# hirofumi0810/tensorflow_end2end_speech_recognition

Hardware: AMD Instinct MI355X
Metric: acoustic frames/sec (train), TIMIT-shaped BLSTM-CTC (higher is better)
Workload: dtype bf16; 1 GPU; TIMIT 61-phone 5x256 BLSTM-CTC, B=16/GPU, D=120, C=62, seq_len~U{100..778}, dropout 0.2, rmsprop, train step; global_batch=16, parallelism=dp1, padded_to=own Tmax per rank

## Files before the change

tensorflow_end2end_speech_recognition_amd/csrc/gemm.hip:

```cpp
#include "common.h"
#include "mfma_tn.h"
#include <stdlib.h>

namespace {

static inline bool first_on_device(unsigned long long& mask) {
  int d = 0;
  (void)hipGetDevice(&d);
  const unsigned long long bit = 1ull << (d & 63);
  if (mask & bit) return false;
  mask |= bit;
  return true;
}

template <typename T> struct GT;
template <> struct GT<float> {
  static constexpr int BK = 32;
  static constexpr int VEC = 4;
};
template <> struct GT<bf16_t> {
  static constexpr int BK = 64;
  static constexpr int VEC = 8;
};

template <typename T> struct Vec16 { T v[GT<T>::VEC]; } __attribute__((aligned(16)));

template <typename TO> __device__ __forceinline__ void store_out(TO* p, float v);
template <> __device__ __forceinline__ void store_out<float>(float* p, float v) { *p = v; }
template <> __device__ __forceinline__ void store_out<bf16_t>(bf16_t* p, float v) { *p = f32_to_bf16(v); }
template <typename TO> __device__ __forceinline__ float load_out(const TO* p);
template <> __device__ __forceinline__ float load_out<float>(const float* p) { return *p; }
template <> __device__ __forceinline__ float load_out<bf16_t>(const bf16_t* p) { return bf16_to_f32(*p); }

template <typename T, int ROWS, bool KCONT>
struct TileLoader {
  static constexpr int BK = GT<T>::BK, VEC = GT<T>::VEC;
  static constexpr int NVEC = ROWS * BK / VEC;
  static constexpr int PER_THREAD = NVEC / 256;
  static_assert(NVEC % 256 == 0, "tile must divide over 256 threads");
  Vec16<T> reg[PER_THREAD];

  __device__ __forceinline__ void load(const T* __restrict__ p, int ld, int r0, int k0, int R,
                                       int K, bool aligned) {
    const int tid = threadIdx.x;
#pragma unroll
    for (int i = 0; i < PER_THREAD; ++i) {
      const int v = tid + i * 256;
      int r, k;
      size_t off;
      int nr, nk;
      if (KCONT) {
        r = v / (BK / VEC); k = (v % (BK / VEC)) * VEC;
        off = (size_t)(r0 + r) * ld + (k0 + k);
        nr = 1; nk = VEC;
      } else {
        k = v / (ROWS / VEC); r = (v % (ROWS / VEC)) * VEC;
        off = (size_t)(k0 + k) * ld + (r0 + r);
        nr = VEC; nk = 1;
      }
      const bool full = (r0 + r + nr <= R) && (k0 + k + nk <= K);
      if (full && aligned) {
        reg[i] = *reinterpret_cast<const Vec16<T>*>(p + off);
      } else {
#pragma unroll
        for (int j = 0; j < VEC; ++j) {
          const int rr = r0 + r + (KCONT ? 0 : j), kk = k0 + k + (KCONT ? j : 0);
          T val = T(0);
          if (rr < R && kk < K) val = p[KCONT ? ((size_t)rr * ld + kk) : ((size_t)kk * ld + rr)];
          reg[i].v[j] = val;
        }
      }
    }
  }
  __device__ __forceinline__ void store(T* s, int lds_ld) const {
    const int tid = threadIdx.x;
#pragma unroll
    for (int i = 0; i < PER_THREAD; ++i) {
      const int v = tid + i * 256;
      if (KCONT) {
        const int r = v / (BK / VEC), k = (v % (BK / VEC)) * VEC;
        *reinterpret_cast<Vec16<T>*>(s + r * lds_ld + k) = reg[i];
      } else {
        const int k = v / (ROWS / VEC), r = (v % (ROWS / VEC)) * VEC;
#pragma unroll
        for (int j = 0; j < VEC; ++j) s[(r + j) * lds_ld + k] = reg[i].v[j];
      }
    }
  }
};

template <typename T, typename TO, int BM, int BN, bool TA, bool TB>
__global__ __launch_bounds__(256) void gemm_kernel(int M, int N, int K, const T* __restrict__ A,
                                                   int lda, const T* __restrict__ B, int ldb,
                                                   TO* __restrict__ C, int ldc,
                                                   const float* __restrict__ bias, int accumulate,
                                                   int a_aligned, int b_aligned, int kchunk,
                                                   float* __restrict__ partial, int act, int c_vec) {
  constexpr int BK = GT<T>::BK, VEC = GT<T>::VEC;
  constexpr int LDS_LD = BK + VEC;
  constexpr int WM = BM / 2, WN = BN / 2, TM = WM / 16, TN = WN / 16;
  extern __shared__ __attribute__((aligned(16))) char smem[];
  T* As = reinterpret_cast<T*>(smem);
  T* Bs = As + BM * LDS_LD;

  const int lane = threadIdx.x & 63, wave = threadIdx.x >> 6;
  const int wm = wave >> 1, wn = wave & 1;
  const int m0 = blockIdx.y * BM, n0 = blockIdx.x * BN;

  TileLoader<T, BM, !TA> la;
  TileLoader<T, BN, TB> lb;

  f32x4_t acc[TM][TN];
#pragma unroll
  for (int i = 0; i < TM; ++i)
#pragma unroll
    for (int j = 0; j < TN; ++j) acc[i][j] = (f32x4_t){0.f, 0.f, 0.f, 0.f};

  const int kbeg = blockIdx.z * kchunk;
  const int kend = min(K, kbeg + kchunk);
  const int nkt = (kend - kbeg + BK - 1) / BK;
  constexpr int STAGE = (BM + BN) * LDS_LD;
  la.load(A, lda, m0, kbeg, M, kend, a_aligned);
  lb.load(B, ldb, n0, kbeg, N, kend, b_aligned);
  la.store(As, LDS_LD);
  lb.store(Bs, LDS_LD);
  __syncthreads();

  for (int kt = 0; kt < nkt; ++kt) {
    const T* Ac = As + (kt & 1) * STAGE;
    const T* Bc = Bs + (kt & 1) * STAGE;
    if (kt + 1 < nkt) {
      la.load(A, lda, m0, kbeg + (kt + 1) * BK, M, kend, a_aligned);
      lb.load(B, ldb, n0, kbeg + (kt + 1) * BK, N, kend, b_aligned);
    }
    const int fr = lane & 15, fq = lane >> 4;
    if constexpr (sizeof(T) == 2) {
#pragma unroll
      for (int ks = 0; ks < BK / 32; ++ks) {
        bf16x8_t a[TM], b[TN];
#pragma unroll
        for (int i = 0; i < TM; ++i)
          a[i] = *reinterpret_cast<const bf16x8_t*>(Ac + (wm * WM + i * 16 + fr) * LDS_LD + ks * 32 + fq * 8);
#pragma unroll
        for (int j = 0; j < TN; ++j)
          b[j] = *reinterpret_cast<const bf16x8_t*>(Bc + (wn * WN + j * 16 + fr) * LDS_LD + ks * 32 + fq * 8);
#pragma unroll
        for (int i = 0; i < TM; ++i)
#pragma unroll
          for (int j = 0; j < TN; ++j)
            acc[i][j] = __builtin_amdgcn_mfma_f32_16x16x32_bf16(b[j], a[i], acc[i][j], 0, 0, 0);
      }
    } else {
#pragma unroll
      for (int ks = 0; ks < BK / 4; ++ks) {
        float a[TM], b[TN];
#pragma unroll
        for (int i = 0; i < TM; ++i) a[i] = Ac[(wm * WM + i * 16 + fr) * LDS_LD + ks * 4 + fq];
#pragma unroll
        for (int j = 0; j < TN; ++j) b[j] = Bc[(wn * WN + j * 16 + fr) * LDS_LD + ks * 4 + fq];
#pragma unroll
        for (int i = 0; i < TM; ++i)
#pragma unroll
          for (int j = 0; j < TN; ++j)
            acc[i][j] = __builtin_amdgcn_mfma_f32_16x16x4f32(b[j], a[i], acc[i][j], 0, 0, 0);
      }
    }
    if (kt + 1 < nkt) {
      la.store(As + ((kt + 1) & 1) * STAGE, LDS_LD);
      lb.store(Bs + ((kt + 1) & 1) * STAGE, LDS_LD);
    }
    __syncthreads();
  }

#pragma unroll
  for (int i = 0; i < TM; ++i)
#pragma unroll
    for (int j = 0; j < TN; ++j) {
      const int m = m0 + wm * WM + i * 16 + (lane & 15);
      const int nb = n0 + wn * WN + j * 16 + (lane >> 4) * 4;
      if (m >= M || nb >= N) continue;
      const bool full = nb + 3 < N;
      if (partial) {
        float* pp = partial + ((size_t)blockIdx.z * M + m) * N + nb;
        if (full && (N & 3) == 0) *reinterpret_cast<f32x4_t*>(pp) = acc[i][j];
        else
          for (int r = 0; r < 4 && nb + r < N; ++r) pp[r] = acc[i][j][r];
        continue;
      }
      TO* cp = C + (size_t)m * ldc + nb;
      float v[4];
#pragma unroll
      for (int r = 0; r < 4; ++r) v[r] = acc[i][j][r] + ((bias && nb + r < N) ? bias[nb + r] : 0.f);
      if (full && c_vec) {
        if constexpr (sizeof(TO) == 4) {
          if (accumulate) {
            const f32x4_t o = *reinterpret_cast<const f32x4_t*>(cp);
#pragma unroll
            for (int r = 0; r < 4; ++r) v[r] += o[r];
          }
          if (act == 1) {
#pragma unroll
            for (int r = 0; r < 4; ++r) v[r] = fmaxf(v[r], 0.f);
          }
          *reinterpret_cast<f32x4_t*>(cp) = (f32x4_t){v[0], v[1], v[2], v[3]};
        } else {
          typedef __attribute__((ext_vector_type(4))) unsigned short us4_t;
          if (accumulate) {
            const us4_t o = *reinterpret_cast<const us4_t*>(cp);
#pragma unroll
            for (int r = 0; r < 4; ++r) v[r] += bf16_to_f32(o[r]);
          }
          if (act == 1) {
#pragma unroll
            for (int r = 0; r < 4; ++r) v[r] = fmaxf(v[r], 0.f);
          }
          *reinterpret_cast<us4_t*>(cp) = (us4_t){f32_to_bf16(v[0]), f32_to_bf16(v[1]), f32_to_bf16(v[2]), f32_to_bf16(v[3])};
        }
      } else {
        for (int r = 0; r < 4 && nb + r < N; ++r) {
          float w = v[r];
          if (accumulate) w += load_out<TO>(cp + r);
          if (act == 1) w = fmaxf(w, 0.f);
          store_out<TO>(cp + r, w);
        }
      }
    }
}

__device__ __forceinline__ unsigned nt_swz(int row) { return (((row + 4) >> 3) & 1) ? 8u : 0u; }

template <bool ANY> __device__ __forceinline__ int nt_tile_of_block(int b, int total) {
  if constexpr (ANY) {
    const int per = total >> 3, rem = total & 7, x = b & 7;
    return x * per + min(x, rem) + (b >> 3);
  } else {
    int t = b;
    if ((total & 7) == 0) t = (t & 7) * (total >> 3) + (t >> 3);
    return t;
  }
}

struct GemmDrop {
  float keep;
  uint64_t seed, offset;
  int use;
};

template <typename TO, bool ROWS = false>
__global__ __launch_bounds__(256) void gemm_nt_bf16_kernel(int M, int N, int K, const bf16_t* __restrict__ A,
                                                           int lda, const bf16_t* __restrict__ Bt, int ldb,
                                                           TO* __restrict__ C, int ldc,
                                                           const float* __restrict__ bias, int accumulate,
                                                           int act, const float* __restrict__ mul, int ldm,
                                                           GemmDrop drop, const int32_t* __restrict__ rows) {
  constexpr int BM = 128, BN = 128, BK = 64, LD = BK + 8;
  constexpr int STAGE = (BM + BN) * LD;
  extern __shared__ __attribute__((aligned(16))) char smem[];
  bf16_t* S = reinterpret_cast<bf16_t*>(smem);

  const int tid = threadIdx.x, lane = tid & 63, wave = tid >> 6;
  const int wm = wave >> 1, wn = wave & 1;
  const int ntn = N / BN, ntm = (M + BM - 1) / BM, total = ntn * ntm;
  const int t = nt_tile_of_block<ROWS>((int)blockIdx.x, total);
  const int m0 = (t / ntn) * BM, n0 = (t % ntn) * BN;

  const bf16_t* pa[4];
  const bf16_t* pb[4];
  unsigned so[4];
#pragma unroll
  for (int i = 0; i < 4; ++i) {
    const int v = tid + i * 256, r = v >> 3, kv = (v & 7) * 8;
    const int ar = min(m0 + r, M - 1);
    pa[i] = A + (size_t)(ROWS ? rows[ar] : ar) * lda + kv;
    pb[i] = Bt + (size_t)(n0 + r) * ldb + kv;
    so[i] = (unsigned)(r * LD) + ((unsigned)kv ^ nt_swz(r));
  }
  bf16x8_t ra[4], rb[4];
  auto gload = [&]() {
#pragma unroll
    for (int i = 0; i < 4; ++i) {
      ra[i] = *reinterpret_cast<const bf16x8_t*>(pa[i]);
      rb[i] = *reinterpret_cast<const bf16x8_t*>(pb[i]);
      pa[i] += BK;
      pb[i] += BK;
    }
  };
  auto sstore = [&](bf16_t* st) {
#pragma unroll
    for (int i = 0; i < 4; ++i) {
      *reinterpret_cast<bf16x8_t*>(st + so[i]) = ra[i];
      *reinterpret_cast<bf16x8_t*>(st + BM * LD + so[i]) = rb[i];
    }
  };

  f32x4_t acc[4][4];
#pragma unroll
  for (int i = 0; i < 4; ++i)
#pragma unroll
    for (int j = 0; j < 4; ++j) acc[i][j] = (f32x4_t){0.f, 0.f, 0.f, 0.f};

  const int nkt = K / BK;
  gload();
  sstore(S);
  __syncthreads();
  const int fr = lane & 15, fq = lane >> 4;
  const unsigned aoff = (unsigned)((wm * 64 + fr) * LD) + ((unsigned)(fq * 8) ^ nt_swz(fr));
  const unsigned boff = (unsigned)(BM * LD + (wn * 64 + fr) * LD) + ((unsigned)(fq * 8) ^ nt_swz(fr));
  for (int kt = 0; kt < nkt; ++kt) {
    const bf16_t* cur = S + (kt & 1) * STAGE;
    if (kt + 1 < nkt) gload();
#pragma unroll
    for (int ks = 0; ks < 2; ++ks) {
      bf16x8_t a[4], b[4];
#pragma unroll
      for (int i = 0; i < 4; ++i) a[i] = *reinterpret_cast<const bf16x8_t*>(cur + aoff + i * 16 * LD + ks * 32);
#pragma unroll
      for (int j = 0; j < 4; ++j) b[j] = *reinterpret_cast<const bf16x8_t*>(cur + boff + j * 16 * LD + ks * 32);
#pragma unroll
      for (int i = 0; i < 4; ++i)
#pragma unroll
        for (int j = 0; j < 4; ++j)
          acc[i][j] = __builtin_amdgcn_mfma_f32_16x16x32_bf16(b[j], a[i], acc[i][j], 0, 0, 0);
    }
    if (kt + 1 < nkt) sstore(S + ((kt + 1) & 1) * STAGE);
    __syncthreads();
  }
#pragma unroll
  for (int i = 0; i < 4; ++i) {
    const int mi = m0 + wm * 64 + i * 16 + fr;
    if (mi >= M) continue;
    const int m = ROWS ? rows[mi] : mi;
#pragma unroll
    for (int j = 0; j < 4; ++j) {
      const int nb = n0 + wn * 64 + j * 16 + fq * 4;
      TO* cp = C + (size_t)m * ldc + nb;
      float v[4];
#pragma unroll
      for (int r = 0; r < 4; ++r) v[r] = acc[i][j][r];
      if (bias) {
        const f32x4_t bv = *reinterpret_cast<const f32x4_t*>(bias + nb);
#pragma unroll
        for (int r = 0; r < 4; ++r) v[r] += bv[r];
      }
      if constexpr (sizeof(TO) == 4) {
        if (accumulate) {
          const f32x4_t o = *reinterpret_cast<const f32x4_t*>(cp);
#pragma unroll
          for (int r = 0; r < 4; ++r) v[r] += o[r];
        }
        if (act == 1) {
#pragma unroll
          for (int r = 0; r < 4; ++r) v[r] = fmaxf(v[r], 0.f);
        }
        if (mul) {
          const f32x4_t mv = *reinterpret_cast<const f32x4_t*>(mul + (size_t)m * ldm + nb);
#pragma unroll
          for (int r = 0; r < 4; ++r) v[r] *= mv[r];
        }
        if (drop.use) {
          float mk[4];
          asr_dropout_words(drop.offset + ((size_t)m * N + nb) / 4, drop.seed, drop.keep, 1.f / drop.keep, mk);
#pragma unroll
          for (int r = 0; r < 4; ++r) v[r] *= mk[r];
        }
        *reinterpret_cast<f32x4_t*>(cp) = (f32x4_t){v[0], v[1], v[2], v[3]};
      } else {
        typedef __attribute__((ext_vector_type(4))) unsigned short us4_t;
        if (accumulate) {
          const us4_t o = *reinterpret_cast<const us4_t*>(cp);
#pragma unroll
          for (int r = 0; r < 4; ++r) v[r] += bf16_to_f32(o[r]);
        }
        if (act == 1) {
#pragma unroll
          for (int r = 0; r < 4; ++r) v[r] = fmaxf(v[r], 0.f);
        }
        *reinterpret_cast<us4_t*>(cp) = (us4_t){f32_to_bf16(v[0]), f32_to_bf16(v[1]), f32_to_bf16(v[2]), f32_to_bf16(v[3])};
      }
    }
  }
}

template <typename TO, int BM, int BN, int WM, int WN, bool ROWS = false>
__global__ __launch_bounds__(WM * WN * 64, 1) void gemm_nt_bf16_big_kernel(int M, int N, int K, const bf16_t* __restrict__ A,
                                                                           int lda, const bf16_t* __restrict__ Bt, int ldb,
                                                                           TO* __restrict__ C, int ldc,
                                                                           const float* __restrict__ bias, int accumulate,
                                                                           int act, const float* __restrict__ mul, int ldm,
                                                                           GemmDrop drop, const int32_t* __restrict__ rows) {
  constexpr int BK = 64, LD = BK + 8, NT = WM * WN * 64;
  constexpr int STAGE = (BM + BN) * LD;
  constexpr int TM = BM / WM, TN = BN / WN, TI = TM / 16, TJ = TN / 16;
  constexpr int VA = BM * 8 / NT, VB = BN * 8 / NT, RSTEP = NT / 8;
  extern __shared__ __attribute__((aligned(16))) char smem[];
  bf16_t* S = reinterpret_cast<bf16_t*>(smem);

  const int tid = threadIdx.x, lane = tid & 63, wave = tid >> 6;
  const int wm = wave / WN, wn = wave % WN;
  const int ntn = N / BN, ntm = (M + BM - 1) / BM, total = ntn * ntm;
  const int t = nt_tile_of_block<ROWS>((int)blockIdx.x, total);
  const int m0 = (t / ntn) * BM, n0 = (t % ntn) * BN;

  const int r0 = tid >> 3, kv = (tid & 7) * 8;
  unsigned oa[VA], ob[VB];
#pragma unroll
  for (int i = 0; i < VA; ++i) {
    const int ar = min(m0 + r0 + RSTEP * i, M - 1);
    oa[i] = (unsigned)(((size_t)(ROWS ? rows[ar] : ar) * lda + kv) * sizeof(bf16_t));
  }
#pragma unroll
  for (int i = 0; i < VB; ++i) ob[i] = (unsigned)(((size_t)(n0 + r0 + RSTEP * i) * ldb + kv) * sizeof(bf16_t));
  const unsigned so0 = (unsigned)(r0 * LD) + ((unsigned)kv ^ nt_swz(r0));
  const __amdgpu_buffer_rsrc_t rsA = __builtin_amdgcn_make_buffer_rsrc(
      const_cast<bf16_t*>(A), 0,
      (int)min((size_t)0xFFFFFFFFu, ((size_t)(ROWS ? rows[M - 1] : M - 1) * lda + K) * sizeof(bf16_t)), 0x00020000);
  const __amdgpu_buffer_rsrc_t rsB = __builtin_amdgcn_make_buffer_rsrc(
      const_cast<bf16_t*>(Bt), 0, (int)min((size_t)0xFFFFFFFFu, ((size_t)(N - 1) * ldb + K) * sizeof(bf16_t)), 0x00020000);
  typedef __attribute__((ext_vector_type(4))) unsigned u32x4_t;
  u32x4_t ra[VA], rb[VB];
  unsigned koff = 0;
  auto gload = [&]() {
#pragma unroll
    for (int i = 0; i < VA; ++i) ra[i] = __builtin_amdgcn_raw_buffer_load_b128(rsA, oa[i], koff, 0);
#pragma unroll
    for (int i = 0; i < VB; ++i) rb[i] = __builtin_amdgcn_raw_buffer_load_b128(rsB, ob[i], koff, 0);
    koff += BK * sizeof(bf16_t);
  };
  auto sstore = [&](bf16_t* st) {
#pragma unroll
    for (int i = 0; i < VA; ++i) *reinterpret_cast<u32x4_t*>(st + so0 + i * RSTEP * LD) = ra[i];
#pragma unroll
    for (int i = 0; i < VB; ++i) *reinterpret_cast<u32x4_t*>(st + BM * LD + so0 + i * RSTEP * LD) = rb[i];
  };

  f32x4_t acc[TI][TJ];
#pragma unroll
  for (int i = 0; i < TI; ++i)
#pragma unroll
    for (int j = 0; j < TJ; ++j) acc[i][j] = (f32x4_t){0.f, 0.f, 0.f, 0.f};

  const int nkt = K / BK;
  gload();
  sstore(S);
  __syncthreads();
  const int fr = lane & 15, fq = lane >> 4;
  const unsigned aoff = (unsigned)((wm * TM + fr) * LD) + ((unsigned)(fq * 8) ^ nt_swz(fr));
  const unsigned boff = (unsigned)(BM * LD + (wn * TN + fr) * LD) + ((unsigned)(fq * 8) ^ nt_swz(fr));
  for (int kt = 0; kt < nkt; ++kt) {
    const bf16_t* cur = S + (kt & 1) * STAGE;
    if (kt + 1 < nkt) gload();
#pragma unroll
    for (int ks = 0; ks < 2; ++ks) {
      bf16x8_t a[TI];
#pragma unroll
      for (int i = 0; i < TI; ++i) a[i] = *reinterpret_cast<const bf16x8_t*>(cur + aoff + i * 16 * LD + ks * 32);
#pragma unroll
      for (int jh = 0; jh < TJ; jh += 4) {
        bf16x8_t b[4];
#pragma unroll
        for (int j = 0; j < 4; ++j) b[j] = *reinterpret_cast<const bf16x8_t*>(cur + boff + (jh + j) * 16 * LD + ks * 32);
#pragma unroll
        for (int i = 0; i < TI; ++i)
#pragma unroll
          for (int j = 0; j < 4; ++j)
            acc[i][jh + j] = __builtin_amdgcn_mfma_f32_16x16x32_bf16(b[j], a[i], acc[i][jh + j], 0, 0, 0);
      }
    }
    if (kt + 1 < nkt) sstore(S + ((kt + 1) & 1) * STAGE);
    __syncthreads();
  }
#pragma unroll
  for (int i = 0; i < TI; ++i) {
    const int mi = m0 + wm * TM + i * 16 + fr;
    if (mi >= M) continue;
    const int m = ROWS ? rows[mi] : mi;
#pragma unroll
    for (int j = 0; j < TJ; ++j) {
      const int nb = n0 + wn * TN + j * 16 + fq * 4;
      TO* cp = C + (size_t)m * ldc + nb;
      float v[4];
#pragma unroll
      for (int r = 0; r < 4; ++r) v[r] = acc[i][j][r];
      if (bias) {
        const f32x4_t bv = *reinterpret_cast<const f32x4_t*>(bias + nb);
#pragma unroll
        for (int r = 0; r < 4; ++r) v[r] += bv[r];
      }
      if constexpr (sizeof(TO) == 4) {
        if (accumulate) {
          const f32x4_t o = *reinterpret_cast<const f32x4_t*>(cp);
#pragma unroll
          for (int r = 0; r < 4; ++r) v[r] += o[r];
        }
        if (act == 1) {
#pragma unroll
          for (int r = 0; r < 4; ++r) v[r] = fmaxf(v[r], 0.f);
        }
        if (mul) {
          const f32x4_t mv = *reinterpret_cast<const f32x4_t*>(mul + (size_t)m * ldm + nb);
#pragma unroll
          for (int r = 0; r < 4; ++r) v[r] *= mv[r];
        }
        if (drop.use) {
          float mk[4];
          asr_dropout_words(drop.offset + ((size_t)m * N + nb) / 4, drop.seed, drop.keep, 1.f / drop.keep, mk);
#pragma unroll
          for (int r = 0; r < 4; ++r) v[r] *= mk[r];
        }
        *reinterpret_cast<f32x4_t*>(cp) = (f32x4_t){v[0], v[1], v[2], v[3]};
      } else {
        typedef __attribute__((ext_vector_type(4))) unsigned short us4_t;
        if (accumulate) {
          const us4_t o = *reinterpret_cast<const us4_t*>(cp);
#pragma unroll
          for (int r = 0; r < 4; ++r) v[r] += bf16_to_f32(o[r]);
        }
        if (act == 1) {
#pragma unroll
          for (int r = 0; r < 4; ++r) v[r] = fmaxf(v[r], 0.f);
        }
        *reinterpret_cast<us4_t*>(cp) = (us4_t){f32_to_bf16(v[0]), f32_to_bf16(v[1]), f32_to_bf16(v[2]), f32_to_bf16(v[3])};
      }
    }
  }
}

template <typename TO, int BM, int BN, int WM, int WN, bool ROWS = false>
static void launch_gemm_nt_big(int M, int N, int K, const void* A, int lda, const void* B, int ldb, void* C, int ldc,
                               const float* bias, int accumulate, hipStream_t st, int act, const float* mul, int ldm,
                               GemmDrop drop, const int32_t* rows = nullptr) {
  const size_t lds = (size_t)2 * (BM + BN) * (64 + 8) * sizeof(bf16_t);
  static unsigned long long attr_done = 0;
  auto k = gemm_nt_bf16_big_kernel<TO, BM, BN, WM, WN, ROWS>;
  if (first_on_device(attr_done)) {
    (void)hipFuncSetAttribute((const void*)k, hipFuncAttributeMaxDynamicSharedMemorySize, (int)lds);
  }
  const long tiles = (long)(N / BN) * ((M + BM - 1) / BM);
  hipLaunchKernelGGL(k, dim3((unsigned)tiles), dim3(WM * WN * 64), lds, st, M, N, K, (const bf16_t*)A, lda,
                     (const bf16_t*)B, ldb, (TO*)C, ldc, bias, accumulate, act, mul, ldm, drop, rows);
}

static void launch_gemm_nt_rows128(int nrows, int N, int K, const void* A, int lda, const void* B, int ldb, float* C,
                                   int ldc, const float* bias, int accumulate, hipStream_t st, int act,
                                   const float* mul, int ldm, GemmDrop drop, const int32_t* rows) {
  const size_t lds = (size_t)2 * (128 + 128) * (64 + 8) * sizeof(bf16_t);
  static unsigned long long attr_done = 0;
  auto k = gemm_nt_bf16_kernel<float, true>;
  if (first_on_device(attr_done)) {
    (void)hipFuncSetAttribute((const void*)k, hipFuncAttributeMaxDynamicSharedMemorySize, (int)lds);
  }
  const int total = (N / 128) * ((nrows + 127) / 128);
  hipLaunchKernelGGL(k, dim3(total), dim3(256), lds, st, nrows, N, K, (const bf16_t*)A, lda, (const bf16_t*)B, ldb, C,
                     ldc, bias, accumulate, act, mul, ldm, drop, rows);
}

template <typename TO>
bool try_gemm_nt_bf16(int transA, int transB, int M, int N, int K, const void* A, int lda, const void* B,
                      int ldb, void* C, int ldc, const float* bias, int accumulate, hipStream_t st, int act,
                      const float* mul, int ldm, GemmDrop drop = GemmDrop{1.f, 0, 0, 0}, const int32_t* rows = nullptr,
                      int nrows = 0, unsigned long long* counts = nullptr) {
  if (transA || !transB || K % 64 != 0 || N % 128 != 0 || M < 1024) return false;
  if (drop.use && sizeof(TO) != 4) return false;
  if (mul && (sizeof(TO) != 4 || ldm % 4 != 0 || ((uintptr_t)mul) % 16 != 0)) return false;
  if (lda % 8 != 0 || ldb % 8 != 0 || ((uintptr_t)A) % 16 != 0 || ((uintptr_t)B) % 16 != 0) return false;
  if (ldc % 4 != 0 || ((uintptr_t)C) % (4 * sizeof(TO)) != 0 || (bias && ((uintptr_t)bias) % 16 != 0)) return false;
  if (rows && (sizeof(TO) != 4 || nrows < 1 || nrows > M)) return false;
  static const int big = [] { const char* e = getenv("ASR_GEMM_NT_BIG"); return e ? atoi(e) : 1; }();
  const bool fits32 = ((size_t)(M - 1) * lda + K) * sizeof(bf16_t) < 0xFFFFFFFFull && ((size_t)(N - 1) * ldb + K) * sizeof(bf16_t) < 0xFFFFFFFFull;
  const int Mk = rows ? nrows : M;
  const long tiles256 = (long)(N / 256) * ((Mk + 255) / 256);
  const bool use_big = big && fits32 && N % 256 == 0 && (big == 2 ? Mk >= 2048 : tiles256 >= 512);
  if constexpr (sizeof(TO) == 4) {
    if (rows) {
      if (use_big)
        launch_gemm_nt_big<float, 256, 256, 2, 4, true>(Mk, N, K, A, lda, B, ldb, C, ldc, bias, accumulate, st, act, mul,
                                                         ldm, drop, rows);
      else
        launch_gemm_nt_rows128(Mk, N, K, A, lda, B, ldb, (float*)C, ldc, bias, accumulate, st, act, mul, ldm, drop, rows);
      if (counts) counts[use_big ? ASR_GEMMP_ROWS_256 : ASR_GEMMP_ROWS_128] += 1;
      return true;
    }
  }
  if (use_big) {
    launch_gemm_nt_big<TO, 256, 256, 2, 4>(M, N, K, A, lda, B, ldb, C, ldc, bias, accumulate, st, act, mul, ldm, drop);
    return true;
  }
  const size_t lds = (size_t)2 * (128 + 128) * (64 + 8) * sizeof(bf16_t);
  static unsigned long long attr_done = 0;
  if (first_on_device(attr_done)) {
    (void)hipFuncSetAttribute((const void*)gemm_nt_bf16_kernel<TO>, hipFuncAttributeMaxDynamicSharedMemorySize, (int)lds);
  }
  const int total = (N / 128) * ((M + 127) / 128);
  hipLaunchKernelGGL(gemm_nt_bf16_kernel<TO>, dim3(total), dim3(256), lds, st, M, N, K, (const bf16_t*)A, lda,
                     (const bf16_t*)B, ldb, (TO*)C, ldc, bias, accumulate, act, mul, ldm, drop, (const int32_t*)nullptr);
  return true;
}

__device__ __forceinline__ int xcd_work_index(int skip) {
  const int b = blockIdx.x, x = b & 7;
  if (x < skip) return -1;
  return (b >> 3) * (8 - skip) + (x - skip);
}
static inline unsigned xcd_grid(long work, int skip) {
  const long per = 8 - skip;
  return (unsigned)((work + per - 1) / per * 8);
}

constexpr int SK_WAVES = 8;
struct SkinnyCell {
  const float *c_prev, *h_prev, *peep, *live, *out_mask;
  float *gates, *c_raw, *c_out, *h_out, *h_raw, *cell_out, *h_out2, *cell_out2;
  int U, ld_h2, ld_c2;
  float fb, clip;
};
__device__ __forceinline__ float sk_sigf(float x) { return 1.0f / (1.0f + expf(-x)); }
template <bool TRANSB, int NT, bool CELL = false, bool BH = false>
__global__ __launch_bounds__(64 * SK_WAVES) void gemm_skinny_f32_kernel(int M, int N, int K, const float* __restrict__ A,
                                                                        int lda, const float* __restrict__ Bm, int ldb,
                                                                        float* __restrict__ C, int ldc,
                                                                        const float* __restrict__ bias, int accumulate,
                                                                        int act, SkinnyCell cell) {
  constexpr int TN = 16 * NT;
  __shared__ float red[SK_WAVES][16][TN + 1];
  const int lane = threadIdx.x & 63, wave = threadIdx.x >> 6;
  const int col = lane & 15, rg = lane >> 4;
  const int n0 = blockIdx.x * TN, m0 = blockIdx.y * 16;
  float cl_cp = 0.f, cl_hp = 0.f, cl_lv = 0.f, cl_wci = 0.f, cl_wcf = 0.f, cl_wco = 0.f, cl_om = 1.f;
  const int cl_m = m0 + (int)threadIdx.x / (TN / 4), cl_u = n0 / 4 + (int)threadIdx.x % (TN / 4);
  const bool cl_on = CELL && (int)threadIdx.x < 16 * (TN / 4) && cl_m < M;
  if (CELL && cl_on) {
    const size_t ci = (size_t)cl_m * cell.U + cl_u;
    cl_cp = cell.c_prev[ci];
    cl_hp = cell.h_prev[ci];
    cl_lv = cell.live[cl_m];
    if (cell.peep) { cl_wci = cell.peep[cl_u]; cl_wcf = cell.peep[cell.U + cl_u]; cl_wco = cell.peep[2 * cell.U + cl_u]; }
    if (cell.out_mask) cl_om = cell.out_mask[ci];
  }
  typedef __attribute__((ext_vector_type(4))) unsigned skw4_t;
  static_assert(!BH || (TRANSB ? NT == 1 : NT == 2), "bf16 weights: NT = 2 fragment image / NT = 1 transposed rows");
  struct Frag {
    f32x4_t a[4], b[BH ? 1 : NT][BH ? 1 : 4];
    skw4_t w[BH ? (TRANSB ? 2 : 4) : 1];
    float keep;
  };
  f32x4_t acc[NT];
#pragma unroll
  for (int j = 0; j < NT; ++j) acc[j] = (f32x4_t){0.f, 0.f, 0.f, 0.f};
  const float* ap = A + (size_t)min(m0 + col, M - 1) * lda + ((BH && TRANSB) ? rg * 16 : rg * 4);
  const int units = K / 64;
  const bf16_t* Bh = reinterpret_cast<const bf16_t*>(Bm);
  auto load = [&](int round, Frag& f) {
    const int unit = wave + round * SK_WAVES;
    const bool valid = unit < units;
    const int kb = (valid ? unit : units - 1) * 64;
    f.keep = valid ? 1.f : 0.f;
    if constexpr (BH) {
      if constexpr (TRANSB) {
#pragma unroll
        for (int j = 0; j < 4; ++j) f.a[j] = *reinterpret_cast<const f32x4_t*>(ap + kb + j * 4);
        const bf16_t* bp = Bh + (size_t)(n0 + col) * ldb + kb + rg * 16;
        f.w[0] = *reinterpret_cast<const skw4_t*>(bp);
        f.w[1] = *reinterpret_cast<const skw4_t*>(bp + 8);
      } else {
#pragma unroll
        for (int j = 0; j < 4; ++j) f.a[j] = *reinterpret_cast<const f32x4_t*>(ap + kb + j * 16);
        const skw4_t* bp = reinterpret_cast<const skw4_t*>(Bh + (((size_t)blockIdx.x * units + (kb >> 6)) * 64 + lane) * 32);
#pragma unroll
        for (int j = 0; j < 4; ++j) f.w[j] = bp[j];
      }
      return;
    }
#pragma unroll
    for (int j = 0; j < 4; ++j) {
      f.a[j] = *reinterpret_cast<const f32x4_t*>(ap + kb + j * 16);
#pragma unroll
      for (int n = 0; n < NT; ++n) {
        if (TRANSB) {
          f.b[n][j] = *reinterpret_cast<const f32x4_t*>(Bm + (size_t)(n0 + n * 16 + col) * ldb + kb + j * 16 + rg * 4);
        } else {
          const float* bp = Bm + (size_t)(kb + j * 16 + rg * 4) * ldb + n0 + n * 16 + col;
#pragma unroll
          for (int e = 0; e < 4; ++e) f.b[n][j][e] = bp[(size_t)e * ldb];
        }
      }
    }
  };
  auto mma = [&](const Frag& f) {
    if constexpr (BH) {
#pragma unroll
      for (int j = 0; j < 4; ++j)
#pragma unroll
        for (int e = 0; e < 4; ++e) {
          if constexpr (TRANSB) {
            const int t = 4 * j + e;
            const unsigned wd = f.w[t >> 3][(t & 7) >> 1];
            const float bv = __uint_as_float((t & 1) ? (wd & 0xffff0000u) : (wd << 16));
            acc[0] = __builtin_amdgcn_mfma_f32_16x16x4f32(f.a[j][e] * f.keep, bv, acc[0], 0, 0, 0);
          } else {
            const unsigned wd = f.w[j][e];
            acc[0] = __builtin_amdgcn_mfma_f32_16x16x4f32(f.a[j][e] * f.keep, __uint_as_float(wd << 16), acc[0], 0, 0, 0);
            acc[NT - 1] = __builtin_amdgcn_mfma_f32_16x16x4f32(f.a[j][e] * f.keep, __uint_as_float(wd & 0xffff0000u), acc[NT - 1], 0, 0, 0);
          }
        }
      return;
    }
#pragma unroll
    for (int j = 0; j < 4; ++j)
#pragma unroll
      for (int e = 0; e < 4; ++e)
#pragma unroll
        for (int n = 0; n < NT; ++n)
          acc[n] = __builtin_amdgcn_mfma_f32_16x16x4f32(f.a[j][e] * f.keep, f.b[n][j][e], acc[n], 0, 0, 0);
  };
  Frag f0, f1;
  load(0, f0);
  if (units <= SK_WAVES) {
    mma(f0);
  } else {
    const int rounds = ((units + SK_WAVES - 1) / SK_WAVES + 1) & ~1;
    for (int r = 0; r < rounds; r += 2) {
      load(r + 1, f1);
      __builtin_amdgcn_sched_barrier(0);
      mma(f0);
      __builtin_amdgcn_sched_barrier(0);
      load(r + 2, f0);
      __builtin_amdgcn_sched_barrier(0);
      mma(f1);
      __builtin_amdgcn_sched_barrier(0);
    }
  }
#pragma unroll
  for (int n = 0; n < NT; ++n)
#pragma unroll
    for (int r = 0; r < 4; ++r) red[wave][rg * 4 + r][n * 16 + col] = acc[n][r];
  __syncthreads();
  if constexpr (CELL) {
    if (!cl_on) return;
    const int m = (int)threadIdx.x / (TN / 4), ul = (int)threadIdx.x % (TN / 4), U = cell.U;
    float p[4];
#pragma unroll
    for (int g = 0; g < 4; ++g) {
      float v = 0.f;
#pragma unroll
      for (int w = 0; w < SK_WAVES; ++w) v += red[w][m][ul * 4 + g];
      if (bias) v += bias[n0 + ul * 4 + g];
      p[g] = v;
    }
    const float cp = cl_cp;
    const float i = sk_sigf(p[0] + cl_wci * cp);
    const float g = tanhf(p[1]);
    const float f = sk_sigf(p[2] + cell.fb + cl_wcf * cp);
    float cn = g * i + cp * f;
    if (cell.clip > 0.f) cn = fminf(fmaxf(cn, -cell.clip), cell.clip);
    const float o = sk_sigf(p[3] + cl_wco * cn);
    const float hn = tanhf(cn) * o;
    const size_t ci = (size_t)cl_m * U + cl_u;
    float* gp = cell.gates + (size_t)cl_m * 4 * U;
    gp[cl_u] = i; gp[U + cl_u] = g; gp[2 * U + cl_u] = f; gp[3 * U + cl_u] = o;
    cell.c_raw[ci] = cn;
    cell.h_raw[ci] = hn;
    cell.c_out[ci] = cl_lv > 0.f ? cn : cp;
    const float ho = cl_lv > 0.f ? hn : cl_hp;
    cell.h_out[ci] = ho;
    if (cell.h_out2) cell.h_out2[(size_t)cl_m * cell.ld_h2 + cl_u] = ho;
    const float co = cell.out_mask ? hn * cl_om : hn;
    if (cell.cell_out) cell.cell_out[ci] = co;
    if (cell.cell_out2) cell.cell_out2[(size_t)cl_m * cell.ld_c2 + cl_u] = co;
    return;
  }
  for (int idx = threadIdx.x; idx < 16 * TN; idx += 64 * SK_WAVES) {
    const int m = idx / TN, n = idx % TN;
    if (m0 + m >= M) continue;
    float v = 0.f;
#pragma unroll
    for (int w = 0; w < SK_WAVES; ++w) v += red[w][m][n];
    if (bias) v += bias[n0 + n];
    float* cp = C + (size_t)(m0 + m) * ldc + n0 + n;
    if (accumulate) v += *cp;
    if (act == 1) v = fmaxf(v, 0.f);
    *cp = v;
  }
}

static bool try_gemm_skinny_f32(int transA, int transB, int M, int N, int K, const void* A, int lda, const void* B,
                                int ldb, void* C, int ldc, const float* bias, int accumulate, hipStream_t st, int act) {
  if (transA || M < 1 || M > 32 || K % 64 != 0 || N % 16 != 0 || K < 64) return false;
  if (lda % 4 != 0 || ((uintptr_t)A) % 16 != 0 || ((uintptr_t)B) % 16 != 0) return false;
  if (transB && ldb % 4 != 0) return false;
  const bool wide = (N % 32 == 0) && (!transB || N >= 32 * 192);
  const unsigned gy = (unsigned)((M + 15) / 16);
#define ASR_SKINNY(TB, NT_)                                                                                             \
  hipLaunchKernelGGL((gemm_skinny_f32_kernel<TB, NT_>), dim3(N / (16 * NT_), gy), dim3(64 * SK_WAVES), 0, st, M, N, K, \
                     (const float*)A, lda, (const float*)B, ldb, (float*)C, ldc, bias, accumulate, act, SkinnyCell{})
  if (transB) {
    if (wide) ASR_SKINNY(true, 2); else ASR_SKINNY(true, 1);
  } else {
    if (wide) ASR_SKINNY(false, 2); else ASR_SKINNY(false, 1);
  }
#undef ASR_SKINNY
  return true;
}

__global__ __launch_bounds__(256) void gemm_tn_bf16_kernel(int M, int N, int K, const bf16_t* __restrict__ A,
                                                           int lda, const bf16_t* __restrict__ Bm, int ldb,
                                                           int kchunk, float* __restrict__ partial, int tn, int tm,
                                                           int nslab, int xcd_skip) {
  constexpr int BM = 128, BN = 128, BK = 64;
  extern __shared__ __attribute__((aligned(16))) char smem[];

  const int widx = xcd_work_index(xcd_skip);
  if (widx < 0 || widx >= tn * tm * nslab) return;
  const int bx = widx % tn, by = (widx / tn) % tm, bz = widx / (tn * tm);
  const int tid = threadIdx.x, lane = tid & 63, wave = tid >> 6;
  const int wm = wave >> 1, wn = wave & 1;
  const int m0 = by * BM, n0 = bx * BN;
  const int kbeg = bz * kchunk, kend = min(K, kbeg + kchunk);
  const int nkt = (kend - kbeg + BK - 1) / BK;

  const int mvec = tid & 15, kr0 = tid >> 4;
  const bool a_ok = m0 + mvec * 8 + 8 <= M, b_ok = n0 + mvec * 8 + 8 <= N;
  const bf16_t* pa = A + (size_t)(kbeg + kr0) * lda + m0 + mvec * 8;
  const bf16_t* pb = Bm + (size_t)(kbeg + kr0) * ldb + n0 + mvec * 8;
  const bf16x8_t zero = {0, 0, 0, 0, 0, 0, 0, 0};
  bf16x8_t ra[4], rb[4];
  auto gload = [&](int kt) {
#pragma unroll
    for (int q = 0; q < 4; ++q) {
      const int k = kbeg + kt * BK + kr0 + 16 * q;
      const size_t ro = (size_t)(kt * BK + 16 * q);
      ra[q] = (a_ok && k < kend) ? *reinterpret_cast<const bf16x8_t*>(pa + ro * lda) : zero;
      rb[q] = (b_ok && k < kend) ? *reinterpret_cast<const bf16x8_t*>(pb + ro * ldb) : zero;
    }
  };
  const unsigned wbase = (unsigned)(mvec >> 1) * TN_SUB + (unsigned)kr0 * 32u + (unsigned)(mvec & 1) * 16u;
  auto sstore = [&](char* st) {
#pragma unroll
    for (int q = 0; q < 4; ++q) {
      *reinterpret_cast<bf16x8_t*>(st + wbase + q * 16 * 32) = ra[q];
      *reinterpret_cast<bf16x8_t*>(st + TN_OPER + wbase + q * 16 * 32) = rb[q];
    }
  };

  f32x4_t acc[4][4];
#pragma unroll
  for (int i = 0; i < 4; ++i)
#pragma unroll
    for (int j = 0; j < 4; ++j) acc[i][j] = (f32x4_t){0.f, 0.f, 0.f, 0.f};

  if (nkt > 0) {
    gload(0);
    sstore(smem);
  }
  __syncthreads();
  const int fr = lane & 15, fq = lane >> 4;
  const unsigned piece = (unsigned)(8 * fq + (fr >> 2)) * 32u + (unsigned)(fr & 3) * 8u;
  unsigned aoff[4], boff[4];
#pragma unroll
  for (int i = 0; i < 4; ++i) {
    aoff[i] = (unsigned)(wm * 4 + i) * TN_SUB + piece;
    boff[i] = (unsigned)TN_OPER + (unsigned)(wn * 4 + i) * TN_SUB + piece;
  }
  for (int kt = 0; kt < nkt; ++kt) {
    const char* cur = smem + (kt & 1) * TN_STAGE;
    if (kt + 1 < nkt) gload(kt + 1);
#pragma unroll
    for (int ks = 0; ks < 2; ++ks) {
      bf16x8_t a[4], b[4];
#pragma unroll
      for (int i = 0; i < 4; ++i) a[i] = tn_frag(cur + aoff[i] + ks * 32 * 32);
#pragma unroll
      for (int j = 0; j < 4; ++j) b[j] = tn_frag(cur + boff[j] + ks * 32 * 32);
#pragma unroll
      for (int i = 0; i < 4; ++i)
#pragma unroll
        for (int j = 0; j < 4; ++j)
          acc[i][j] = __builtin_amdgcn_mfma_f32_16x16x32_bf16(b[j], a[i], acc[i][j], 0, 0, 0);
    }
    if (kt + 1 < nkt) sstore(smem + ((kt + 1) & 1) * TN_STAGE);
    __syncthreads();
  }
  float* slab = partial + (size_t)bz * M * N;
#pragma unroll
  for (int i = 0; i < 4; ++i) {
    const int m = m0 + wm * 64 + i * 16 + fr;
    if (m >= M) continue;
#pragma unroll
    for (int j = 0; j < 4; ++j) {
      const int nb = n0 + wn * 64 + j * 16 + fq * 4;
      if (nb >= N) continue;
      *reinterpret_cast<f32x4_t*>(slab + (size_t)m * N + nb) = acc[i][j];
    }
  }
}


template <typename TO>
__global__ void splitk_reduce_kernel(const float* __restrict__ partial, int S, int M, int N,
// ... 389 lines not shown
```

Measured before the change: 734,200 frames/s.

## Software-pipeline LDS fragment reads in NT GEMM and use BM=64 tiles for small grids

Adds a pipelined variant of the 128x128 NT bf16 GEMM. It double-buffers register fragments across the two k-substeps, issues the global load two tiles ahead, and uses a raw s_barrier with an explicit lgkmcnt wait so LDS reads overlap the MFMAs. When the 128-row tile count is below the CU count, it switches to a BM=64 tile to fill more CUs. An environment variable selects the mode, and the pipelined path is the default. The gain is better latency hiding and occupancy on the mid-size GEMMs, at the cost of extra VGPRs for the second fragment set and a hand-managed barrier that could hide ordering bugs.

After: 737,300 frames/s, median of 6. No clear change (+0.4%).

```diff
diff --git a/tensorflow_end2end_speech_recognition_amd/csrc/gemm.hip b/tensorflow_end2end_speech_recognition_amd/csrc/gemm.hip
--- a/tensorflow_end2end_speech_recognition_amd/csrc/gemm.hip
+++ b/tensorflow_end2end_speech_recognition_amd/csrc/gemm.hip
@@ -246,15 +246,17 @@
   int use;
 };
 
-template <typename TO, bool ROWS = false>
+template <typename TO, bool ROWS = false, int BM = 128, bool PIPE = false>
 __global__ __launch_bounds__(256) void gemm_nt_bf16_kernel(int M, int N, int K, const bf16_t* __restrict__ A,
                                                            int lda, const bf16_t* __restrict__ Bt, int ldb,
                                                            TO* __restrict__ C, int ldc,
                                                            const float* __restrict__ bias, int accumulate,
                                                            int act, const float* __restrict__ mul, int ldm,
                                                            GemmDrop drop, const int32_t* __restrict__ rows) {
-  constexpr int BM = 128, BN = 128, BK = 64, LD = BK + 8;
+  static_assert(BM == 128 || BM == 64, "2 x 2 waves of (BM / 2) x 64");
+  constexpr int BN = 128, BK = 64, LD = BK + 8;
   constexpr int STAGE = (BM + BN) * LD;
+  constexpr int TM = BM / 2, TI = TM / 16, VA = BM / 32;
   extern __shared__ __attribute__((aligned(16))) char smem[];
   bf16_t* S = reinterpret_cast<bf16_t*>(smem);
 
@@ -264,70 +266,113 @@
   const int t = nt_tile_of_block<ROWS>((int)blockIdx.x, total);
   const int m0 = (t / ntn) * BM, n0 = (t % ntn) * BN;
 
-  const bf16_t* pa[4];
+  const bf16_t* pa[VA];
   const bf16_t* pb[4];
   unsigned so[4];
 #pragma unroll
   for (int i = 0; i < 4; ++i) {
     const int v = tid + i * 256, r = v >> 3, kv = (v & 7) * 8;
-    const int ar = min(m0 + r, M - 1);
-    pa[i] = A + (size_t)(ROWS ? rows[ar] : ar) * lda + kv;
+    if (i < VA) {
+      const int ar = min(m0 + r, M - 1);
+      pa[i] = A + (size_t)(ROWS ? rows[ar] : ar) * lda + kv;
+    }
     pb[i] = Bt + (size_t)(n0 + r) * ldb + kv;
     so[i] = (unsigned)(r * LD) + ((unsigned)kv ^ nt_swz(r));
   }
-  bf16x8_t ra[4], rb[4];
+  bf16x8_t ra[VA], rb[4];
   auto gload = [&]() {
 #pragma unroll
     for (int i = 0; i < 4; ++i) {
-      ra[i] = *reinterpret_cast<const bf16x8_t*>(pa[i]);
+      if (i < VA) ra[i] = *reinterpret_cast<const bf16x8_t*>(pa[i]);
       rb[i] = *reinterpret_cast<const bf16x8_t*>(pb[i]);
-      pa[i] += BK;
+      if (i < VA) pa[i] += BK;
       pb[i] += BK;
     }
   };
   auto sstore = [&](bf16_t* st) {
 #pragma unroll
     for (int i = 0; i < 4; ++i) {
-      *reinterpret_cast<bf16x8_t*>(st + so[i]) = ra[i];
+      if (i < VA) *reinterpret_cast<bf16x8_t*>(st + so[i]) = ra[i];
       *reinterpret_cast<bf16x8_t*>(st + BM * LD + so[i]) = rb[i];
     }
   };
 
-  f32x4_t acc[4][4];
-#pragma unroll
-  for (int i = 0; i < 4; ++i)
+  f32x4_t acc[TI][4];
+#pragma unroll
+  for (int i = 0; i < TI; ++i)
 #pragma unroll
     for (int j = 0; j < 4; ++j) acc[i][j] = (f32x4_t){0.f, 0.f, 0.f, 0.f};
 
   const int nkt = K / BK;
-  gload();
-  sstore(S);
-  __syncthreads();
-  const int fr = lane & 15, fq = lane >> 4;
-  const unsigned aoff = (unsigned)((wm * 64 + fr) * LD) + ((unsigned)(fq * 8) ^ nt_swz(fr));
-  const unsigned boff = (unsigned)(BM * LD + (wn * 64 + fr) * LD) + ((unsigned)(fq * 8) ^ nt_swz(fr));
-  for (int kt = 0; kt < nkt; ++kt) {
-    const bf16_t* cur = S + (kt & 1) * STAGE;
-    if (kt + 1 < nkt) gload();
-#pragma unroll
-    for (int ks = 0; ks < 2; ++ks) {
-      bf16x8_t a[4], b[4];
-#pragma unroll
-      for (int i = 0; i < 4; ++i) a[i] = *reinterpret_cast<const bf16x8_t*>(cur + aoff + i * 16 * LD + ks * 32);
-#pragma unroll
-      for (int j = 0; j < 4; ++j) b[j] = *reinterpret_cast<const bf16x8_t*>(cur + boff + j * 16 * LD + ks * 32);
-#pragma unroll
-      for (int i = 0; i < 4; ++i)
+  if constexpr (!PIPE) {
+    gload();
+    sstore(S);
+    __syncthreads();
+    const int fr = lane & 15, fq = lane >> 4;
+    const unsigned aoff = (unsigned)((wm * TM + fr) * LD) + ((unsigned)(fq * 8) ^ nt_swz(fr));
+    const unsigned boff = (unsigned)(BM * LD + (wn * 64 + fr) * LD) + ((unsigned)(fq * 8) ^ nt_swz(fr));
+    for (int kt = 0; kt < nkt; ++kt) {
+      const bf16_t* cur = S + (kt & 1) * STAGE;
+      if (kt + 1 < nkt) gload();
+#pragma unroll
+      for (int ks = 0; ks < 2; ++ks) {
+        bf16x8_t a[TI], b[4];
+#pragma unroll
+        for (int i = 0; i < TI; ++i) a[i] = *reinterpret_cast<const bf16x8_t*>(cur + aoff + i * 16 * LD + ks * 32);
+#pragma unroll
+        for (int j = 0; j < 4; ++j) b[j] = *reinterpret_cast<const bf16x8_t*>(cur + boff + j * 16 * LD + ks * 32);
+#pragma unroll
+        for (int i = 0; i < TI; ++i)
+#pragma unroll
+          for (int j = 0; j < 4; ++j)
+            acc[i][j] = __builtin_amdgcn_mfma_f32_16x16x32_bf16(b[j], a[i], acc[i][j], 0, 0, 0);
+      }
+      if (kt + 1 < nkt) sstore(S + ((kt + 1) & 1) * STAGE);
+      __syncthreads();
+    }
+  } else {
+    const int fr = lane & 15, fq = lane >> 4;
+    const unsigned aoff = (unsigned)((wm * TM + fr) * LD) + ((unsigned)(fq * 8) ^ nt_swz(fr));
+    const unsigned boff = (unsigned)(BM * LD + (wn * 64 + fr) * LD) + ((unsigned)(fq * 8) ^ nt_swz(fr));
+    bf16x8_t a0[TI], b0[4], a1[TI], b1[4];
+    auto fread = [&](bf16x8_t* a, bf16x8_t* b, const bf16_t* buf, int ks) {
+#pragma unroll
+      for (int i = 0; i < TI; ++i) a[i] = *reinterpret_cast<const bf16x8_t*>(buf + aoff + i * 16 * LD + ks * 32);
+#pragma unroll
+      for (int j = 0; j < 4; ++j) b[j] = *reinterpret_cast<const bf16x8_t*>(buf + boff + j * 16 * LD + ks * 32);
+    };
+    auto mma = [&](const bf16x8_t* a, const bf16x8_t* b) {
+#pragma unroll
+      for (int i = 0; i < TI; ++i)
 #pragma unroll
         for (int j = 0; j < 4; ++j)
           acc[i][j] = __builtin_amdgcn_mfma_f32_16x16x32_bf16(b[j], a[i], acc[i][j], 0, 0, 0);
-    }
-    if (kt + 1 < nkt) sstore(S + ((kt + 1) & 1) * STAGE);
+    };
+    gload();
+    sstore(S);
+    if (nkt > 1) gload();
     __syncthreads();
-  }
-#pragma unroll
-  for (int i = 0; i < 4; ++i) {
-    const int mi = m0 + wm * 64 + i * 16 + fr;
+    fread(a0, b0, S, 0);
+    for (int kt = 0; kt < nkt; ++kt) {
+      const bf16_t* cur = S + (kt & 1) * STAGE;
+      bf16_t* nxt = S + ((kt + 1) & 1) * STAGE;
+      fread(a1, b1, cur, 1);
+      if (kt + 1 < nkt) sstore(nxt);
+      if (kt + 2 < nkt) gload();
+      mma(a0, b0);
+      __builtin_amdgcn_sched_barrier(0);
+      asm volatile("s_waitcnt lgkmcnt(0)" ::: "memory");
+      __builtin_amdgcn_s_barrier();
+      asm volatile("" ::: "memory");
+      __builtin_amdgcn_sched_barrier(0);
+      fread(a0, b0, nxt, 0);
+      mma(a1, b1);
+    }
+  }
+  const int fr = lane & 15, fq = lane >> 4;
+#pragma unroll
+  for (int i = 0; i < TI; ++i) {
+    const int mi = m0 + wm * TM + i * 16 + fr;
     if (mi >= M) continue;
     const int m = ROWS ? rows[mi] : mi;
 #pragma unroll
@@ -540,18 +585,42 @@
                      (const bf16_t*)B, ldb, (TO*)C, ldc, bias, accumulate, act, mul, ldm, drop, rows);
 }
 
-static void launch_gemm_nt_rows128(int nrows, int N, int K, const void* A, int lda, const void* B, int ldb, float* C,
-                                   int ldc, const float* bias, int accumulate, hipStream_t st, int act,
-                                   const float* mul, int ldm, GemmDrop drop, const int32_t* rows) {
-  const size_t lds = (size_t)2 * (128 + 128) * (64 + 8) * sizeof(bf16_t);
+template <typename TO, bool ROWS, int BM, bool PIPE>
+static void launch_gemm_nt_lean(int M, int N, int K, const void* A, int lda, const void* B, int ldb, void* C, int ldc,
+                                const float* bias, int accumulate, hipStream_t st, int act, const float* mul, int ldm,
+                                GemmDrop drop, const int32_t* rows) {
+  const size_t lds = (size_t)2 * (BM + 128) * (64 + 8) * sizeof(bf16_t);
   static unsigned long long attr_done = 0;
-  auto k = gemm_nt_bf16_kernel<float, true>;
+  auto k = gemm_nt_bf16_kernel<TO, ROWS, BM, PIPE>;
   if (first_on_device(attr_done)) {
     (void)hipFuncSetAttribute((const void*)k, hipFuncAttributeMaxDynamicSharedMemorySize, (int)lds);
   }
-  const int total = (N / 128) * ((nrows + 127) / 128);
-  hipLaunchKernelGGL(k, dim3(total), dim3(256), lds, st, nrows, N, K, (const bf16_t*)A, lda, (const bf16_t*)B, ldb, C,
+  const int total = (N / 128) * ((M + BM - 1) / BM);
+  hipLaunchKernelGGL(k, dim3(total), dim3(256), lds, st, M, N, K, (const bf16_t*)A, lda, (const bf16_t*)B, ldb, (TO*)C,
                      ldc, bias, accumulate, act, mul, ldm, drop, rows);
+}
+
+static int nt_num_cu() {
+  static int cus[64] = {0};
+  int d = 0;
+  (void)hipGetDevice(&d);
+  int& c = cus[d & 63];
+  if (c == 0 && hipDeviceGetAttribute(&c, hipDeviceAttributeMultiprocessorCount, d) != hipSuccess) c = 0;
+  return c;
+}
+
+template <typename TO, bool ROWS>
+static void launch_gemm_nt_lean_any(int Mk, int N, int K, const void* A, int lda, const void* B, int ldb, void* C, int ldc,
+                                    const float* bias, int accumulate, hipStream_t st, int act, const float* mul, int ldm,
+                                    GemmDrop drop, const int32_t* rows) {
+  static const int mode = [] { const char* e = getenv("ASR_GEMM_NT_PIPE"); const int m = e ? atoi(e) : 1; return m < 0 || m > 2 ? 1 : m; }();
+  const long tiles128 = (long)(N / 128) * ((Mk + 127) / 128);
+#define ASR_NT_LEAN(BM_, PIPE_) \
+  launch_gemm_nt_lean<TO, ROWS, BM_, PIPE_>(Mk, N, K, A, lda, B, ldb, C, ldc, bias, accumulate, st, act, mul, ldm, drop, rows)
+  if (mode == 0) ASR_NT_LEAN(128, false);
+  else if (mode == 1 && tiles128 < nt_num_cu()) ASR_NT_LEAN(64, true);
+  else ASR_NT_LEAN(128, true);
+#undef ASR_NT_LEAN
 }
 
 template <typename TO>
@@ -576,7 +645,7 @@
         launch_gemm_nt_big<float, 256, 256, 2, 4, true>(Mk, N, K, A, lda, B, ldb, C, ldc, bias, accumulate, st, act, mul,
                                                          ldm, drop, rows);
       else
-        launch_gemm_nt_rows128(Mk, N, K, A, lda, B, ldb, (float*)C, ldc, bias, accumulate, st, act, mul, ldm, drop, rows);
+        launch_gemm_nt_lean_any<float, true>(Mk, N, K, A, lda, B, ldb, C, ldc, bias, accumulate, st, act, mul, ldm, drop, rows);
       if (counts) counts[use_big ? ASR_GEMMP_ROWS_256 : ASR_GEMMP_ROWS_128] += 1;
       return true;
     }
@@ -585,14 +654,7 @@
     launch_gemm_nt_big<TO, 256, 256, 2, 4>(M, N, K, A, lda, B, ldb, C, ldc, bias, accumulate, st, act, mul, ldm, drop);
     return true;
   }
-  const size_t lds = (size_t)2 * (128 + 128) * (64 + 8) * sizeof(bf16_t);
-  static unsigned long long attr_done = 0;
-  if (first_on_device(attr_done)) {
-    (void)hipFuncSetAttribute((const void*)gemm_nt_bf16_kernel<TO>, hipFuncAttributeMaxDynamicSharedMemorySize, (int)lds);
-  }
-  const int total = (N / 128) * ((M + 127) / 128);
-  hipLaunchKernelGGL(gemm_nt_bf16_kernel<TO>, dim3(total), dim3(256), lds, st, M, N, K, (const bf16_t*)A, lda,
-                     (const bf16_t*)B, ldb, (TO*)C, ldc, bias, accumulate, act, mul, ldm, drop, (const int32_t*)nullptr);
+  launch_gemm_nt_lean_any<TO, false>(M, N, K, A, lda, B, ldb, C, ldc, bias, accumulate, st, act, mul, ldm, drop, nullptr);
   return true;
 }
 
```
